# mila-iqia/diffusion_for_multi_scale_molecular_dynamics

Hardware: AMD Instinct MI355X
Metric: sampled structures/sec (1000-step predictor-corrector SDE sampling) (higher is better)
Workload: dtype f32 (per-edge matrix products as split-f16 hi/lo x3 MFMA terms with f32 accumulation: 22-bit products; state, updates, reductions and every other layer in f32)

## Files before the change

### diffusion_for_multi_scale_molecular_dynamics_amd/csrc/mdx_egnn_chain.hip

```cpp
#include <hip/hip_runtime.h>
#include <stdint.h>

#include <type_traits>

#include "../../include/mdx_hip.h"

namespace {

typedef _Float16 half8 __attribute__((ext_vector_type(8)));
typedef _Float16 half2v __attribute__((ext_vector_type(2)));
typedef float f32x16 __attribute__((ext_vector_type(16)));
typedef float f32x4 __attribute__((ext_vector_type(4)));
typedef __attribute__((address_space(3))) char lds_c;
typedef __attribute__((address_space(3))) float lds_f;
typedef __attribute__((address_space(1))) const char gbl_c;

constexpr int kWave = 64;
constexpr int kWaves = 4;
constexpr int kTileEdges = 32 * kWaves;
constexpr int kFastD = 6;
constexpr int kRing = 4;
constexpr int kScaleSlots = MDX_EGNN_CHAIN_MAX_LAYERS + 4;
constexpr int kMaxPositions = MDX_EGNN_CHAIN_MAX_LAYERS + 2;
constexpr int kEnds = kScaleSlots - 1;
// ... 1242 lines not shown
__device__ __forceinline__ float normalize_factor(float r2) { return tanhf(r2) / sqrtf(r2 + 1.0e-16f); }

__global__ __launch_bounds__(256) void egnn_coord_aggregate_kernel(const float* __restrict__ s, const float* __restrict__ coord,
                                                                   const int64_t* __restrict__ edges,
                                                                   const int64_t* __restrict__ offsets,
                                                                   const int64_t* __restrict__ degree, int64_t n_nodes, int D,
                                                                   int mean, int flags, float* __restrict__ out)
{
    const int64_t total = n_nodes * D;
    for (int64_t idx = blockIdx.x * (int64_t)blockDim.x + threadIdx.x; idx < total; idx += (int64_t)gridDim.x * blockDim.x) {
        const int64_t node = idx / D;
        const int k = (int)(idx - node * D);
        const int64_t e0 = offsets[node], deg = degree[node];
        const float ci = coord[idx];
        float acc = 0.0f;
        for (int64_t e = e0; e < e0 + deg; ++e) {
            const int64_t dst = edges[2 * e + 1];
            float diff = ci - coord[dst * D + k];
            if (flags & MDX_EGNN_COORD_NORMALIZE) {
                float r2 = 0.0f;
                for (int j = 0; j < D; ++j) {
                    const float dj = coord[node * D + j] - coord[dst * D + j];
                    r2 += dj * dj;
                }
                diff = normalize_factor(r2) * diff;
            }
            acc += diff * coord_head_value(s[e], flags);
        }
        if (mean && deg > 0) acc = acc / (float)deg;
        out[idx] = ci + acc;
    }
}

__global__ __launch_bounds__(256) void segment_combine_kernel(const float* __restrict__ pieces, const int64_t* __restrict__ offsets,
                                                              const int64_t* __restrict__ degree, int64_t n_nodes, int H,
                                                              int mean, float* __restrict__ out, const float* __restrict__ left,
                                                              int64_t boundary_rows)
{
    const int lane = threadIdx.x % kWave;
    const int64_t wave = (blockIdx.x * (int64_t)blockDim.x + threadIdx.x) / kWave;
    const int64_t n_waves = ((int64_t)gridDim.x * blockDim.x) / kWave;
    const int quads = H >> 2;
    for (int64_t node = wave; node < n_nodes; node += n_waves) {
        const int64_t e0 = offsets[node], deg = degree[node], e1 = e0 + deg;
        const float count = (mean && deg > 0) ? (float)deg : 1.0f;
        const int64_t last_row = ((e1 - 1) & 15) == 15 ? ((e1 - 1) >> 4) : boundary_rows + node;
        for (int q = lane; q < quads; q += kWave) {
            f32x4 acc = {0.0f, 0.0f, 0.0f, 0.0f};
            for (int64_t e = e0 | 15; e < e1 - 1; e += 16) acc += reinterpret_cast<const f32x4*>(pieces + (e >> 4) * H)[q];
            if (deg > 0) acc += reinterpret_cast<const f32x4*>(pieces + last_row * H)[q];
            if (mean) acc = acc / count;
            if (left) {
                reinterpret_cast<f32x4*>(out + node * 2 * H)[q] = reinterpret_cast<const f32x4*>(left + node * H)[q];
                reinterpret_cast<f32x4*>(out + node * 2 * H + H)[q] = acc;
            } else {
                reinterpret_cast<f32x4*>(out + node * H)[q] = acc;
            }
        }
    }
}

__global__ __launch_bounds__(256) void egnn_node_gather_kernel(const float* __restrict__ pieces, const int64_t* __restrict__ offsets,
                                                               const int64_t* __restrict__ degree, int64_t n_nodes, int H,
                                                               int mean_messages, float* __restrict__ out,
                                                               const float* __restrict__ left, int64_t boundary_rows,
                                                               const float* __restrict__ s, const float* __restrict__ coord,
                                                               const int64_t* __restrict__ edges, int D, int mean_coords,
                                                               int flags, float* __restrict__ coord_out)
{
    const int lane = threadIdx.x % kWave;
    const int64_t wave = (blockIdx.x * (int64_t)blockDim.x + threadIdx.x) / kWave;
    const int64_t n_waves = ((int64_t)gridDim.x * blockDim.x) / kWave;
    const int quads = H >> 2;
    for (int64_t node = wave; node < n_nodes; node += n_waves) {
        const int64_t e0 = offsets[node], deg = degree[node], e1 = e0 + deg;
        float part[8] = {0, 0, 0, 0, 0, 0, 0, 0}, ci[8];
#pragma unroll
        for (int k = 0; k < 8; ++k) ci[k] = k < D ? coord[node * D + k] : 0.0f;
        for (int64_t e = e0 + lane; e < e1; e += kWave) {
            const int64_t dst = edges[2 * e + 1];
            const float se = coord_head_value(s[e], flags);
            if (flags & MDX_EGNN_COORD_NORMALIZE) {
                float diff[8], r2 = 0.0f;
#pragma unroll
                for (int k = 0; k < 8; ++k) {
                    diff[k] = k < D ? ci[k] - coord[dst * D + k] : 0.0f;
                    if (k < D) r2 += diff[k] * diff[k];
                }
                const float f = normalize_factor(r2);
#pragma unroll
                for (int k = 0; k < 8; ++k)
                    if (k < D) part[k] += (f * diff[k]) * se;
            } else {
#pragma unroll
                for (int k = 0; k < 8; ++k)
                    if (k < D) part[k] += (ci[k] - coord[dst * D + k]) * se;
            }
        }
        const float count = (mean_messages && deg > 0) ? (float)deg : 1.0f;
        const int64_t last_row = ((e1 - 1) & 15) == 15 ? ((e1 - 1) >> 4) : boundary_rows + node;
        for (int q = lane; pieces && q < quads; q += kWave) {
            f32x4 acc = {0.0f, 0.0f, 0.0f, 0.0f};
            for (int64_t e = e0 | 15; e < e1 - 1; e += 16) acc += reinterpret_cast<const f32x4*>(pieces + (e >> 4) * H)[q];
            if (deg > 0) acc += reinterpret_cast<const f32x4*>(pieces + last_row * H)[q];
            if (mean_messages) acc = acc / count;
            if (left) {
                reinterpret_cast<f32x4*>(out + node * 2 * H)[q] = reinterpret_cast<const f32x4*>(left + node * H)[q];
                reinterpret_cast<f32x4*>(out + node * 2 * H + H)[q] = acc;
            } else {
                reinterpret_cast<f32x4*>(out + node * H)[q] = acc;
            }
        }
#pragma unroll
        for (int k = 0; k < 8; ++k) {
            if (k < D) {
                float v = part[k];
                v += __builtin_bit_cast(float, __builtin_amdgcn_update_dpp(0, __builtin_bit_cast(int, v), 0x111, 0xf, 0xf, false));
                v += __builtin_bit_cast(float, __builtin_amdgcn_update_dpp(0, __builtin_bit_cast(int, v), 0x112, 0xf, 0xf, false));
                v += __builtin_bit_cast(float, __builtin_amdgcn_update_dpp(0, __builtin_bit_cast(int, v), 0x114, 0xf, 0xf, false));
                v += __builtin_bit_cast(float, __builtin_amdgcn_update_dpp(0, __builtin_bit_cast(int, v), 0x118, 0xf, 0xf, false));
                v += __builtin_bit_cast(float, __builtin_amdgcn_update_dpp(0, __builtin_bit_cast(int, v), 0x142, 0xa, 0xf, false));
                v += __builtin_bit_cast(float, __builtin_amdgcn_update_dpp(0, __builtin_bit_cast(int, v), 0x143, 0xc, 0xf, false));
                part[k] = __builtin_bit_cast(float, __builtin_amdgcn_readlane(__builtin_bit_cast(int, v), 63));
            }
        }
        if (lane < D) {
            float total = 0.0f, mine = 0.0f;
#pragma unroll
            for (int k = 0; k < 8; ++k) {
                if (k == lane) { total = part[k]; mine = ci[k]; }
            }
            if (mean_coords && deg > 0) total = total / (float)deg;
            coord_out[node * D + lane] = mine + total;
        }
    }
}

// ... 152 lines not shown
int64_t mdx_egnn_piece_rows(int64_t n_edges, int64_t n_nodes)
{
    if (n_edges < 0 || n_nodes < 0) return -1;
    return ((n_edges + 15) >> 4) + n_nodes;
}

int mdx_segment_combine(const float* pieces, int64_t n_edges, const int64_t* offsets, const int64_t* degree, int64_t n_nodes,
                        int H, int mean, const float* left, float* out, mdx_stream_t stream)
{
    if (n_nodes < 0 || H < 4 || n_edges < 0) return MDX_ERR_INVALID_ARG;
    if (H & 3) return MDX_ERR_UNSUPPORTED;
    if (n_nodes == 0) return MDX_OK;
    if (!pieces || !offsets || !degree || !out) return MDX_ERR_INVALID_ARG;
    int64_t blocks = (n_nodes * kWave + 255) / 256;
    if (blocks > 16384) blocks = 16384;
    hipLaunchKernelGGL(segment_combine_kernel, dim3((unsigned)blocks), dim3(256), 0, reinterpret_cast<hipStream_t>(stream),
                       pieces, offsets, degree, n_nodes, H, mean, out, left, (n_edges + 15) >> 4);
    return hipGetLastError() == hipSuccess ? MDX_OK : MDX_ERR_HIP;
}

int mdx_egnn_node_gather(const float* pieces, int64_t n_edges, const int64_t* offsets, const int64_t* degree, int64_t n_nodes,
                         int H, int mean_messages, const float* left, float* out, const float* edge_scalar, const float* coord,
                         int coord_dimension, const int64_t* edges, int mean_coords, int coord_flags, float* coord_out,
                         mdx_stream_t stream)
{
    if (n_nodes < 0 || H < 4 || n_edges < 0 || coord_dimension < 1) return MDX_ERR_INVALID_ARG;
    if (coord_flags & ~(MDX_EGNN_COORD_NORMALIZE | MDX_EGNN_COORD_TANH)) return MDX_ERR_INVALID_ARG;
    if ((H & 3) || coord_dimension > 8) return MDX_ERR_UNSUPPORTED;
    if (n_nodes == 0) return MDX_OK;
    if (!offsets || !degree || !edge_scalar || !coord || !edges || !coord_out) return MDX_ERR_INVALID_ARG;
    if (pieces ? !out : (out || left)) return MDX_ERR_INVALID_ARG;
    int64_t blocks = (n_nodes * kWave + 255) / 256;
    if (blocks > 16384) blocks = 16384;
    hipLaunchKernelGGL(egnn_node_gather_kernel, dim3((unsigned)blocks), dim3(256), 0, reinterpret_cast<hipStream_t>(stream),
                       pieces, offsets, degree, n_nodes, H, mean_messages, out, left, (n_edges + 15) >> 4, edge_scalar, coord, edges,
                       coord_dimension, mean_coords, coord_flags, coord_out);
    return hipGetLastError() == hipSuccess ? MDX_OK : MDX_ERR_HIP;
}

int mdx_mlp_chain_rows(const mdx_egnn_chain_t* c, const float* x, const float* residual, int64_t n_rows,
                       const int64_t* n_rows_dev, float* out, uint32_t* status, mdx_stream_t stream)
{
    if (!c || n_rows < 0) return MDX_ERR_INVALID_ARG;
    if (c->n_message_layers < 1 || c->n_coord_layers != 0 || (c->precision < 0 || c->precision > 2)) return MDX_ERR_INVALID_ARG;
    if (c->n_message_layers > MDX_EGNN_CHAIN_MAX_LAYERS) return MDX_ERR_UNSUPPORTED;
    if (c->hidden != 32 && c->hidden != 64 && c->hidden != 128 && c->hidden != 256) return MDX_ERR_UNSUPPORTED;
    if (n_rows == 0) return MDX_OK;
    if (!c->weight_image || !c->biases || !x || !out || (c->precision >= 1 && !c->weight_exponents)) return MDX_ERR_INVALID_ARG;
    ChainArgs a{};
    a.image = (const char*)c->weight_image; a.biases = c->biases; a.exps = c->weight_exponents;
    a.act_exps = c->activation_exponents; a.act_max = c->activation_maxima;
    a.n_edges_dev = n_rows_dev; a.n_edges = n_rows; a.n_message = c->n_message_layers; a.n_coord = 0; a.D = 0;
    a.rows_in = x; a.residual = residual; a.rows_out = out; a.status = status; a.ld_in = c->hidden;
    const int layers = a.n_message;
    hipStream_t st = reinterpret_cast<hipStream_t>(stream);
#define MDX_ROWS_CASE(HH)                                                                          \
    case HH: return c->precision == 0 ? launch_chain<HH, 0, 1>(a, layers, st) : (c->precision == 1 ? launch_chain<HH, 1, 1>(a, layers, st) : launch_chain<HH, 2, 1>(a, layers, st));
    switch (c->hidden) {
        MDX_ROWS_CASE(32)
        MDX_ROWS_CASE(64)
        MDX_ROWS_CASE(128)
        MDX_ROWS_CASE(256)
    }
#undef MDX_ROWS_CASE
    return MDX_ERR_UNSUPPORTED;
}

// ... 69 lines not shown
```

### diffusion_for_multi_scale_molecular_dynamics_amd/csrc/mdx_egnn_table.hip

```cpp
#include <hip/hip_runtime.h>
#include <stdint.h>

#include "../../include/mdx_hip.h"
#include "mdx_launch.hpp"

using namespace mdx;

namespace {

typedef float f32x4 __attribute__((ext_vector_type(4)));

__device__ __forceinline__ void lagrange_weights(float t, float w[4])
{
    const float tp = t + 1.0f, tm = t - 1.0f, t2 = t - 2.0f;
    w[0] = -(t * tm * t2) / 6.0f;
    w[1] = (tp * tm * t2) / 2.0f;
    w[2] = -(tp * t * t2) / 2.0f;
    w[3] = (tp * t * tm) / 6.0f;
}

__device__ __forceinline__ float interpolate(const float w[4], float v0, float v1, float v2, float v3)
{
    return ((w[0] * v0 + w[1] * v1) + w[2] * v2) + w[3] * v3;
}

__device__ __forceinline__ f32x4 interpolate4(const float w[4], f32x4 v0, f32x4 v1, f32x4 v2, f32x4 v3)
{
    return ((w[0] * v0 + w[1] * v1) + w[2] * v2) + w[3] * v3;
}

__device__ __forceinline__ float squared_distance(const float* ci, const float* __restrict__ cj, int D)
{
    float r2 = 0.0f;
    for (int k = 0; k < D; ++k) {
        const float dlt = ci[k] - cj[k];
        r2 += dlt * dlt;
    }
    return r2;
}

__device__ __forceinline__ float coord_head_value(float s, int flags) { return (flags & MDX_EGNN_COORD_TANH) ? tanhf(s) : s; }
__device__ __forceinline__ float normalize_factor(float r2) { return tanhf(r2) / sqrtf(r2 + 1.0e-16f); }

__device__ __forceinline__ unsigned abs_bits(float v) { return __float_as_uint(v) & 0x7fffffffu; }

constexpr int kCheckRows = 32;
__global__ __launch_bounds__(256) void egnn_table_check_kernel(const float* __restrict__ messages, const float* __restrict__ scalar,
                                                               int H, int n_pairs, int n_even, unsigned* __restrict__ workspace,
                                                               const uint32_t* __restrict__ table_key,
                                                               const float* __restrict__ sigma)
{
    if (table_is_current(table_key, sigma)) return;
    const int p = blockIdx.x, K = 2 * n_even - 1;
    const int j0 = blockIdx.y * kCheckRows, j1 = min(j0 + kCheckRows, n_even - 2);
    float w[4];
    lagrange_weights(0.5f, w);
    for (int c = threadIdx.x; c <= H; c += blockDim.x) {
        auto value = [&](int row) { return c < H ? messages[((int64_t)p * K + row) * H + c] : scalar[(int64_t)p * K + row]; };
        unsigned err = 0, big = 0;
        for (int j = j0; j < j1; ++j) {
            const float v0 = value(j > 0 ? j - 1 : 1), v1 = value(j), v2 = value(j + 1), v3 = value(j + 2);
            const float mid = value(n_even + j);
            err = max(err, abs_bits(interpolate(w, v0, v1, v2, v3) - mid));
            big = max(big, max(max(abs_bits(v1), abs_bits(v2)), max(abs_bits(v3), abs_bits(mid))));
        }
        if (j0 < j1) {
            atomicMax(workspace + (int64_t)p * (H + 1) + c, err);
            atomicMax(workspace + (int64_t)n_pairs * (H + 1) + p, big);
        }
    }
}
// ... 15 lines not shown
        if (big > 0.0f) mine = fmaxf(mine, err / big);
        else if (err > 0.0f || err != err) mine = INFINITY;
    }
    __syncthreads();
    if (built)
        for (int64_t i = threadIdx.x; i < n_entries + n_pairs; i += blockDim.x) workspace[i] = 0u;
    const int table_fail = fail;
    for (int64_t i = 1 + threadIdx.x; i < n_sigma; i += blockDim.x)
        if (!(sigma[i] == sigma[0])) fail = 1;
    worst[threadIdx.x] = mine;
    bad[threadIdx.x] = fail | (table_fail << 1);
    __syncthreads();
    for (int s = 128; s > 0; s >>= 1) {
        if ((int)threadIdx.x < s) {
            worst[threadIdx.x] = fmaxf(worst[threadIdx.x], worst[threadIdx.x + s]);
            bad[threadIdx.x] |= bad[threadIdx.x + s];
        }
        __syncthreads();
    }
    if (threadIdx.x == 0) {
        if (worst_out && built) worst_out[0] = worst[0];
        if (bad[0] && status) atomicOr(status, MDX_STATUS_EGNN_TABLE);
        if (table_key && built) {
            if (bad[0] & 2) {
                table_key[0] = MDX_EGNN_TABLE_NO_KEY;
            } else {
                table_key[0] = __float_as_uint(sigma[0]);
                table_key[1] = table_key[1] + 1u;
            }
        }
    }
}

__global__ __launch_bounds__(256) void egnn_table_gather_kernel(const float* __restrict__ table, const float* __restrict__ table_scalar,
                                                                int H, int n_classes, int n_even, float inv_spacing,
                                                                const int64_t* __restrict__ atom_types,
                                                                const int64_t* __restrict__ offsets, const int64_t* __restrict__ degree,
                                                                int64_t n_nodes, int mean_messages, float* __restrict__ out,
                                                                const float* __restrict__ left, const float* __restrict__ coord,
                                                                const int64_t* __restrict__ edges, int D, int mean_coords,
                                                                int flags, float* __restrict__ coord_out, uint32_t* __restrict__ status)
{
    const int lane = threadIdx.x % kWave;
    const int64_t wave = (blockIdx.x * (int64_t)blockDim.x + threadIdx.x) / kWave;
    const int64_t n_waves = ((int64_t)gridDim.x * blockDim.x) / kWave;
    const int K = 2 * n_even - 1, quads = H >> 2;
    const bool has_quad = lane < quads;
    bool outside = false;
    for (int64_t node = wave; node < n_nodes; node += n_waves) {
        const int64_t e0 = offsets[node], deg = degree[node], e1 = e0 + deg;
        int64_t a = atom_types[node];
        if (a < 0 || a >= n_classes) { outside = true; a = 0; }
        float part[8] = {0, 0, 0, 0, 0, 0, 0, 0}, ci[8];
#pragma unroll
        for (int k = 0; k < 8; ++k) ci[k] = k < D ? coord[node * D + k] : 0.0f;
        f32x4 acc = {0.0f, 0.0f, 0.0f, 0.0f};
        for (int64_t c0 = e0; c0 < e1; c0 += kWave) {
            const int64_t e = c0 + lane;
            int row = 0, row_left = 0;
            float w[4] = {0, 0, 0, 0};
            if (e < e1) {
                const int64_t dst = edges[2 * e + 1];
                int64_t b = atom_types[dst];
                if (b < 0 || b >= n_classes) { outside = true; b = 0; }
                const float r2 = squared_distance(ci, coord + dst * D, D);
                const float u = sqrtf(r2) * inv_spacing;
                int m = 0;
                float t = 0.0f;
                if (u <= (float)(n_even - 2)) {
                    m = min((int)u, n_even - 3);
                    t = u - (float)m;
                } else {
                    outside = true;
                }
                lagrange_weights(t, w);
                row = (int)(a * n_classes + b) * K + m;
                row_left = m > 0 ? row - 1 : row + 1;
                const float s = coord_head_value(interpolate(w, table_scalar[row_left], table_scalar[row], table_scalar[row + 1],
                                                             table_scalar[row + 2]), flags);
                if (flags & MDX_EGNN_COORD_NORMALIZE) {
                    float diff[8], n2 = 0.0f;
#pragma unroll
                    for (int k = 0; k < 8; ++k) {
                        diff[k] = k < D ? ci[k] - coord[dst * D + k] : 0.0f;
                        if (k < D) n2 += diff[k] * diff[k];
                    }
                    const float f = normalize_factor(n2);
#pragma unroll
                    for (int k = 0; k < 8; ++k)
                        if (k < D) part[k] += (f * diff[k]) * s;
                } else {
#pragma unroll
                    for (int k = 0; k < 8; ++k)
                        if (k < D) part[k] += (ci[k] - coord[dst * D + k]) * s;
                }
            }
            const int n = (int)min<int64_t>(kWave, e1 - c0);
            for (int i = 0; i < n; ++i) {
                const int r = __builtin_amdgcn_readlane(row, i), rl = __builtin_amdgcn_readlane(row_left, i);
                float wi[4];
#pragma unroll
                for (int k = 0; k < 4; ++k)
                    wi[k] = __builtin_bit_cast(float, __builtin_amdgcn_readlane(__builtin_bit_cast(int, w[k]), i));
                if (has_quad) {
                    const f32x4* base = reinterpret_cast<const f32x4*>(table + (int64_t)r * H) + lane;
                    const f32x4 v0 = reinterpret_cast<const f32x4*>(table + (int64_t)rl * H)[lane];
                    acc += interpolate4(wi, v0, base[0], base[quads], base[2 * quads]);
                }
            }
        }
        const float count = (mean_messages && deg > 0) ? (float)deg : 1.0f;
        if (has_quad) {
            if (mean_messages) acc = acc / count;
            if (left) {
                reinterpret_cast<f32x4*>(out + node * 2 * H)[lane] = reinterpret_cast<const f32x4*>(left + node * H)[lane];
                reinterpret_cast<f32x4*>(out + node * 2 * H + H)[lane] = acc;
            } else {
                reinterpret_cast<f32x4*>(out + node * H)[lane] = acc;
            }
        }
#pragma unroll
        for (int k = 0; k < 8; ++k) {
            if (k < D) {
                float v = part[k];
                v += __builtin_bit_cast(float, __builtin_amdgcn_update_dpp(0, __builtin_bit_cast(int, v), 0x111, 0xf, 0xf, false));
                v += __builtin_bit_cast(float, __builtin_amdgcn_update_dpp(0, __builtin_bit_cast(int, v), 0x112, 0xf, 0xf, false));
                v += __builtin_bit_cast(float, __builtin_amdgcn_update_dpp(0, __builtin_bit_cast(int, v), 0x114, 0xf, 0xf, false));
                v += __builtin_bit_cast(float, __builtin_amdgcn_update_dpp(0, __builtin_bit_cast(int, v), 0x118, 0xf, 0xf, false));
                v += __builtin_bit_cast(float, __builtin_amdgcn_update_dpp(0, __builtin_bit_cast(int, v), 0x142, 0xa, 0xf, false));
                v += __builtin_bit_cast(float, __builtin_amdgcn_update_dpp(0, __builtin_bit_cast(int, v), 0x143, 0xc, 0xf, false));
                part[k] = __builtin_bit_cast(float, __builtin_amdgcn_readlane(__builtin_bit_cast(int, v), 63));
            }
        }
        if (lane < D) {
            float total = 0.0f, mine = 0.0f;
#pragma unroll
            for (int k = 0; k < 8; ++k) {
                if (k == lane) { total = part[k]; mine = ci[k]; }
            }
            if (mean_coords && deg > 0) total = total / (float)deg;
// ... 17 lines not shown

int mdx_egnn_table_check_keyed(const float* table, const float* table_scalar, int H, int n_classes, int n_even, const float* sigma,
                               int64_t n_sigma, float tolerance, uint32_t* workspace, float* worst_out, uint32_t* status,
                               uint32_t* table_key, mdx_stream_t stream)
{
    if (H < 1 || n_classes < 1 || n_even < 4 || n_sigma < 1 || !(tolerance >= 0.0f)) return MDX_ERR_INVALID_ARG;
    if (!table || !table_scalar || !sigma || !workspace) return MDX_ERR_INVALID_ARG;
    const int n_pairs = n_classes * n_classes;
    const hipStream_t s = as_stream(stream);
    hipLaunchKernelGGL(egnn_table_check_kernel, dim3((unsigned)n_pairs, (unsigned)((n_even - 2 + kCheckRows - 1) / kCheckRows)),
                       dim3(256), 0, s, table, table_scalar, H, n_pairs, n_even, reinterpret_cast<unsigned*>(workspace),
                       table_key, sigma);
    hipLaunchKernelGGL(egnn_table_verdict_kernel, dim3(1), dim3(256), 0, s, reinterpret_cast<unsigned*>(workspace), n_pairs,
                       H + 1, sigma, n_sigma, tolerance, worst_out, status, table_key);
    return launch_status();
}

int mdx_egnn_table_gather(const float* table, const float* table_scalar, int H, int n_classes, int n_even, float inv_spacing,
                          const int64_t* atom_types, const int64_t* offsets, const int64_t* degree, int64_t n_nodes,
                          int mean_messages, const float* left, float* out, const float* coord, int coord_dimension,
                          const int64_t* edges, int mean_coords, int coord_flags, float* coord_out, uint32_t* status,
                          mdx_stream_t stream)
{
    if (n_nodes < 0 || H < 4 || n_classes < 1 || n_even < 4 || coord_dimension < 1 || !(inv_spacing > 0.0f))
        return MDX_ERR_INVALID_ARG;
    if (coord_flags & ~(MDX_EGNN_COORD_NORMALIZE | MDX_EGNN_COORD_TANH)) return MDX_ERR_INVALID_ARG;
    if ((H & 3) || H > 4 * kWave || coord_dimension > 8) return MDX_ERR_UNSUPPORTED;
    if ((int64_t)n_classes * n_classes * (2 * (int64_t)n_even - 1) * H >= ((int64_t)1 << 31)) return MDX_ERR_UNSUPPORTED;
    if (n_nodes == 0) return MDX_OK;
    if (!table || !table_scalar || !atom_types || !offsets || !degree || !out || !coord || !edges || !coord_out)
        return MDX_ERR_INVALID_ARG;
    int64_t blocks = (n_nodes * kWave + 255) / 256;
    if (blocks > 16384) blocks = 16384;
    hipLaunchKernelGGL(egnn_table_gather_kernel, dim3((unsigned)blocks), dim3(256), 0, as_stream(stream),
                       table, table_scalar, H, n_classes, n_even, inv_spacing, atom_types, offsets, degree, n_nodes, mean_messages,
                       out, left, coord, edges, coord_dimension, mean_coords, coord_flags, coord_out, status);
    return launch_status();
}

}
```

### diffusion_for_multi_scale_molecular_dynamics_amd/models/egnn.py

```python
from typing import Callable, Optional, Tuple

import torch
from torch import nn

from .. import kernels
from ..namespace import AXL


def run_mlp(layers, x: torch.Tensor, fused: bool = False) -> torch.Tensor:
    for layer in layers:
        x = layer(x)
    return x


def segment_sum_sorted(data: torch.Tensor, degree: torch.Tensor) -> torch.Tensor:
    return torch.segment_reduce(data, "sum", lengths=degree, axis=0, unsafe=True)


class LayerDeviceState:
    KINDS = ("edge", "rows", "node")

    def __init__(self):
        self.packs = {kind: {} for kind in self.KINDS}
        self.in_use = {kind: (None, None) for kind in self.KINDS}
# ... 267 lines not shown
                                                table, coords_only)
        assert n_edges is None, "a capacity-sized edge list needs the fused edge chain in every layer"
        count = degree.clamp(min=1).to(h.dtype).unsqueeze(1)

        coord_diff = coord.index_select(0, row) - coord.index_select(0, col)
        radial = (coord_diff ** 2).sum(dim=1, keepdim=True)
        if self.normalize:
            coord_diff = torch.tanh(radial) / torch.sqrt(radial + self.epsilon ** 2) * coord_diff

        messages = self._messages(h, edge_index, radial, fused)

        segments = fused and offsets is not None and messages.shape[1] % 4 == 0
        if segments and self._coord_head_is_plain():
            hidden = run_mlp(list(self.coord_mlp)[:-1], messages, fused)
            coord = coord + kernels.egnn_coord_head(hidden.contiguous(), self.coord_mlp[-1].weight.reshape(-1),
                                                    coord_diff.contiguous(), offsets, degree, self.coords_mean)
        else:
            trans = segment_sum_sorted(coord_diff * run_mlp(self.coord_mlp, messages, fused), degree)
            coord = coord + (trans / count if self.coords_mean else trans)

        if segments:
            agg = kernels.segment_rows(messages.contiguous(), offsets, degree, self.message_mean)
        else:
            agg = segment_sum_sorted(messages, degree)
            if self.message_mean:
                agg = agg / count
        out = run_mlp(self.node_mlp, torch.cat([h, agg], dim=1), fused)
        if self.residual:
            out = h + out
        return out, coord


    def table_applies(self, pack, h, coord) -> bool:
        return (pack is not None and not self.attention and pack.piece_sums_ok and pack.message_width == pack.hidden
                and pack.hidden <= 256 and h.shape[1] == pack.hidden and coord.shape[1] <= 8 and self.status_word is not None
                and h.shape[0] < (1 << 31))

    def _table_gather(self, pack, table, left, coord, edge_index, offsets, degree):
        _, grid_coord, grid_edges = kernels.egnn_table_grid(table.n_classes, table.n_even, coord.shape[1], coord.device)
        memo = table.memo
        values, scalars = kernels.egnn_edge_chain(pack, memo.grid_proj, grid_coord, grid_edges, status=self.status_word,
                                                  memo=memo, sigma=table.sigma)
        self.device_state.table_worst = memo.worst
        kernels.egnn_table_check(values, scalars, table.n_classes, table.n_even, table.sigma, memo.workspace,
                                 worst=memo.worst, status=self.status_word, key=memo.key)
        return kernels.egnn_table_gather(values, scalars, table.n_classes, table.n_even, table.atom_types, offsets, degree,
                                         self.message_mean, left, coord, edge_index, self.coords_mean,
                                         flags=self._coord_flags(), status=self.status_word)

    def _forward_edge_chain(self, pack, h, edge_index, coord, degree, offsets, n_edges=None, node_proj=None, next_layer=None,
                            table=None, coords_only=False):
        coord = coord.contiguous()
        if table is not None and self.table_applies(pack, h, coord):
            def gather(left):
                return self._table_gather(pack, table, left, coord, edge_index, offsets, degree)
            return self._node_part(h, gather, next_layer)
        proj = node_proj if node_proj is not None else torch.nn.functional.linear(h, pack.proj_weight)
        in_kernel = pack.piece_sums_ok and h.shape[0] < (1 << 31)
        messages, edge_scalar = kernels.egnn_edge_chain(pack, proj.contiguous(), coord, edge_index, status=self.status_word,
                                                        n_edges_dev=n_edges, piece_sums=in_kernel)
        padded = pack.message_width != pack.hidden
        if padded:
            coord_out = kernels.egnn_coord_aggregate(edge_scalar, coord, edge_index, offsets, degree, self.coords_mean,
                                                     flags=self._coord_flags())
            agg = (kernels.segment_combine(messages, edge_index.shape[0], offsets, degree, self.message_mean) if in_kernel
                   else kernels.segment_rows(messages, offsets, degree, self.message_mean))
            node_in = torch.cat([h, agg[:, :pack.message_width]], dim=1)
        elif in_kernel and h.shape[1] == messages.shape[1] and coord.shape[1] <= 8:
            if coords_only and not self.attention:
# ... 97 lines not shown
```

### diffusion_for_multi_scale_molecular_dynamics_amd/models/score_networks/egnn_score_network.py

```python
import itertools
import math
from dataclasses import dataclass
from typing import AnyStr, Callable, Dict, Optional, Union

import torch

from ...namespace import AXL, NOISE, NOISY_AXL_COMPOSITION
from ...utils import neighbors
from ..egnn import EGNN
from .score_network import ScoreNetwork, ScoreNetworkParameters


@dataclass(kw_only=True)
class EGNNScoreNetworkParameters(ScoreNetworkParameters):

    architecture: str = "egnn"
    number_of_bloch_wave_shells: int = 1
    message_n_hidden_dimensions: int = 1
    message_hidden_dimensions_size: int = 16
    node_n_hidden_dimensions: int = 1
    node_hidden_dimensions_size: int = 32
    coordinate_n_hidden_dimensions: int = 1
    coordinate_hidden_dimensions_size: int = 32
    residual: bool = True
# ... 42 lines not shown


class EGNNScoreNetwork(ScoreNetwork):

    def __init__(self, hyper_params: EGNNScoreNetworkParameters, edge_builder: Optional[Callable] = None):
        super().__init__(hyper_params)
        hp = hyper_params
        self.number_of_features_per_node = self.num_atom_types + 2
        self.number_of_bloch_wave_shells = hp.number_of_bloch_wave_shells
        k_vectors = positive_bloch_wave_vectors(hp.number_of_bloch_wave_shells, self.spatial_dimension)
        self.register_parameter("bloch_wave_reciprocal_lattice_vectors",
                                torch.nn.Parameter(k_vectors, requires_grad=False))
        self.register_parameter("projection_matrices",
                                torch.nn.Parameter(self._projection_matrices(k_vectors), requires_grad=False))
        assert hp.edges in ("fully_connected", "radial_cutoff"), \
            f"Edges type should be fully_connected or radial_cutoff. Got {hp.edges}"
        self.edges = hp.edges
        self.radial_cutoff = hp.radial_cutoff
        if self.edges == "fully_connected":
            assert self.radial_cutoff is None, "Specifying a radial cutoff is inconsistent with edges=fully_connected."
        else:
            assert type(self.radial_cutoff) is float, \
                "A floating point value for the radial cutoff is needed for edges=radial_cutoff."
        self.drop_duplicate_edges = hp.drop_duplicate_edges
        self.edge_builder = edge_builder
        self.graph_status = None
        self.static_edge_list_max_fraction = 0.5
        self._logged_two_call_switch = False
        self.first_layer_table = "auto"
        self.sigma_uniform_hint = False
        self.first_layer_table_reuse = True
        self.skip_unread_logits = True
        self.logits_unread_hint = False
        self.egnn = self._make_egnn(hp)

    def __getstate__(self):
        state = dict(self.__dict__)
        state.pop("_fully_connected_edges", None)
        state.pop("_table_grid_x", None)
        return state

    @property
    def edge_chain_precision(self):
        return self.egnn.graph_layers[0].edge_chain_precision if len(self.egnn.graph_layers) else None

    @edge_chain_precision.setter
    def edge_chain_precision(self, value):
        for layer in self.egnn.graph_layers:
            layer.edge_chain_precision = value

    def adapt_f16_range(self):
        for layer in self.egnn.graph_layers:
            layer.adapt_f16_range()

    def begin_f16_range_fallback(self):
        for layer in self.egnn.graph_layers:
            layer.begin_f16_range_fallback()

    def reset_f16_range(self):
        for layer in self.egnn.graph_layers:
            layer.reset_f16_range()

    def table_builds(self) -> int:
        return self.egnn.graph_layers[0].table_builds() if len(self.egnn.graph_layers) else 0

    def check_status(self):
        if self.graph_status is not None:
            try:
                neighbors._raise_if_cutoff_too_large(self.graph_status)
            finally:
                self.graph_status.zero_()

    def _impose_non_mask_atomic_type_prediction(self, output: AXL):
        if output.A is not None and not getattr(output.A, "_mdx_mask_imposed", False):
            super()._impose_non_mask_atomic_type_prediction(output)

    def _first_projection_of_inputs(self):
        from ... import kernels
        layers = self.egnn.graph_layers
        if len(layers) == 0 or not layers[0].use_fused_ops:
            return None
        pack = layers[0]._edge_chain_pack()
        emb = self.egnn.embedding_in
        if pack is None or pack.proj_weight.shape[1] != emb.out_features:
            return None
        first = layers[0].message_mlp[0].weight
        stamp = kernels.parameter_stamp(first, emb.weight, emb.bias) + (layers[0].edge_chain_precision,)
        if getattr(self, "_first_projection", (None, None))[0] != stamp:
            with torch.no_grad():
                w2 = (pack.proj_weight.double() @ emb.weight.double()).float().contiguous()
                b2 = (pack.proj_weight.double() @ emb.bias.double()).float().contiguous()
            self._first_projection = (stamp, (w2, b2))
        return self._first_projection[1]

    def _first_layer_table(self, edges, z, h, sigma, atom_types, k_vectors, second):
        from ... import kernels
        mode = self.first_layer_table
        if mode not in ("auto", "on", "off"):
            raise ValueError(f"first_layer_table should be auto, on or off. Got {mode}")
        layer = self.egnn.graph_layers[0]
        if mode != self.__dict__.get("_table_mode_seen", mode):
            layer.reset_table_memos()
        self._table_mode_seen = mode
        if mode == "off" or (mode == "auto" and not self.sigma_uniform_hint):
            return None
        if not layer.table_applies(layer._edge_chain_pack(), h, z):
            return None
        n_classes = self.num_atom_types + 1
        n_even = kernels.egnn_table_points(z.shape[1])
        if mode == "auto" and n_classes ** 2 * (2 * n_even - 1) * 8 > edges.shape[0]:
            return None
        classes, _, _ = kernels.egnn_table_grid(n_classes, n_even, z.shape[1], z.device)
        G = classes.shape[0]
        grid_x = self.__dict__.get("_table_grid_x")
        if grid_x is None or grid_x.shape[1] != G or grid_x.device != z.device:
            grid_x = self._table_grid_x = torch.zeros(1, G, 3, dtype=torch.float32, device=z.device)
        sigma = sigma.to(device=z.device, dtype=torch.float32).reshape(-1).contiguous()
        emb = self.egnn.embedding_in
        stamp = kernels.parameter_stamp(emb.weight, emb.bias, *second)
        memo = layer.table_memo(layer._edge_chain_pack(), n_classes, n_even, emb.out_features, z.shape[1], z.device, stamp)
        if not self.first_layer_table_reuse:
            memo.reset()
        _, _, grid_proj = kernels.egnn_node_inputs(grid_x, k_vectors.contiguous(), sigma, classes.reshape(1, G),
                                                   emb.weight.detach().contiguous(), emb.bias.detach().contiguous(), second=second,
                                                   memo=memo)
        return kernels.EgnnTable(grid_proj=grid_proj, sigma=sigma, atom_types=atom_types.reshape(-1).long().contiguous(),
                                 n_classes=n_classes, n_even=n_even, memo=memo)

    def _make_egnn(self, hp):
        return EGNN(
            input_size=self.number_of_features_per_node, num_classes=self.num_atom_types + 1,
            message_n_hidden_dimensions=hp.message_n_hidden_dimensions,
            message_hidden_dimensions_size=hp.message_hidden_dimensions_size,
            node_n_hidden_dimensions=hp.node_n_hidden_dimensions,
            node_hidden_dimensions_size=hp.node_hidden_dimensions_size,
            coordinate_n_hidden_dimensions=hp.coordinate_n_hidden_dimensions,
            coordinate_hidden_dimensions_size=hp.coordinate_hidden_dimensions_size,
            residual=hp.residual, attention=hp.attention, normalize=hp.normalize, tanh=hp.tanh,
            coords_agg=hp.coords_agg, message_agg=hp.message_agg, n_layers=hp.n_layers)

    @staticmethod
    def _projection_matrices(k_vectors: torch.Tensor) -> torch.Tensor:
        n_k, d = k_vectors.shape
        gamma = torch.zeros(d, 2 * n_k, 2 * n_k)
# ... 46 lines not shown
        if not fits and not self._logged_two_call_switch:
            import logging
            logging.getLogger(__name__).warning(
                "EGNN radius graph: a capacity-sized edge list would take %.1f GB of the %.1f GB free on the device; using "
                "the two-call protocol (one host read per forward, the sampler iteration is not captured in a hipGraph)",
                needed / 2 ** 30, free / 2 ** 30)
            self._logged_two_call_switch = True
        return fits

    def capture_safe(self, batch_size: int, number_of_atoms: int, device) -> bool:
        if self.edges == "fully_connected":
            return True
        if self.edge_builder is not None:
            return False
        return self._static_edge_list_fits(batch_size, number_of_atoms, torch.device(device))

    def _forward_unchecked(self, batch: Dict[AnyStr, torch.Tensor], conditional: bool = False) -> AXL:
        comp = batch[NOISY_AXL_COMPOSITION]
        x = comp.X
        bsz, n, d = x.shape
        if x.is_cuda and (self.graph_status is None or self.graph_status.device != x.device):
            self.graph_status = torch.zeros(1, dtype=torch.int32, device=x.device)
        for layer in self.egnn.graph_layers:
            layer.status_word = self.graph_status if x.is_cuda else None
        edges, degree = self._build_edges(x, comp.L)

        emb = self.egnn.embedding_in
        sigma_in = batch[NOISE]
        if (x.is_cuda and not torch.is_grad_enabled() and d == 3 and x.dtype == torch.float32 and
                emb.in_features == self.num_atom_types + 2 and sigma_in.numel() == bsz):
            from ... import kernels
            k_vectors = self.bloch_wave_reciprocal_lattice_vectors.to(x)
            second = self._first_projection_of_inputs()
            res = kernels.egnn_node_inputs(x.contiguous(), k_vectors.contiguous(),
                                           sigma_in.to(device=x.device, dtype=torch.float32).reshape(-1).contiguous(),
                                           comp.A.reshape(bsz, n).long().contiguous(), emb.weight.detach().contiguous(),
                                           emb.bias.detach().contiguous(), second=second)
            z, h, first_proj = res if second is not None else (res[0], res[1], None)
            table = self._first_layer_table(edges, z, h, sigma_in, comp.A, k_vectors, second) if second is not None else None
            head = self.egnn.node_classification_layer
            if head.out_features <= 8 and head.in_features % 4 == 0 and comp.L.dtype == torch.float32:
                out = self.egnn(h=h, edges=edges, x=z, degree=degree, embedded=True, first_proj=first_proj, classify=False,
                                first_table=table, coords_only=self.skip_unread_logits and self.logits_unread_hint)
                if out.A is None:
                    scores = kernels.egnn_scores(z, out.X.contiguous(), k_vectors.contiguous())
                    return AXL(A=None, X=scores.reshape(bsz, n, d), L=torch.zeros_like(comp.L))
                scores, logits, zeros = kernels.egnn_outputs(
                    z, out.X.contiguous(), k_vectors.contiguous(), out.A.contiguous(), head.weight.detach().contiguous(),
                    head.bias.detach().contiguous(), self.num_atom_types, comp.L.numel())
                logits = logits.reshape(bsz, n, -1)
                logits._mdx_mask_imposed = True
                return AXL(A=logits, X=scores.reshape(bsz, n, d), L=zeros.reshape(comp.L.shape))
            out = self.egnn(h=h, edges=edges, x=z, degree=degree, embedded=True, first_proj=first_proj, first_table=table)
            scores = kernels.egnn_scores(z, out.X.contiguous(), k_vectors.contiguous())
            return AXL(A=out.A.reshape(bsz, n, -1), X=scores.reshape(bsz, n, d), L=torch.zeros_like(comp.L))

        flat = x.reshape(bsz * n, d)
        k_vectors = self.bloch_wave_reciprocal_lattice_vectors.to(flat)
        if flat.is_cuda:
            kr = ((2.0 * math.pi * flat)[:, None, :] * k_vectors[None, :, :]).sum(dim=-1)
        else:
            kr = (2.0 * math.pi * flat) @ k_vectors.t()
        if flat.is_cuda:
            kr64 = kr.double()
            z = torch.stack([kr64.cos().to(kr.dtype), kr64.sin().to(kr.dtype)], dim=2).reshape(bsz * n, -1)
        else:
            z = torch.stack([kr.cos(), kr.sin()], dim=2).reshape(bsz * n, -1)

        sigmas = batch[NOISE].to(x.device).repeat_interleave(n, dim=0)
        one_hot = torch.nn.functional.one_hot(comp.A.reshape(-1).long(), self.num_atom_types + 1).to(x.dtype)
        h = torch.cat([sigmas, one_hot], dim=1)
# ... 9 lines not shown
```

Baseline: 21.64.

## Batch piece loads, specialize gather kernels for D=6, skip dead first projections

```diff
diff --git a/diffusion_for_multi_scale_molecular_dynamics_amd/csrc/mdx_egnn_chain.hip b/diffusion_for_multi_scale_molecular_dynamics_amd/csrc/mdx_egnn_chain.hip
--- a/diffusion_for_multi_scale_molecular_dynamics_amd/csrc/mdx_egnn_chain.hip
+++ b/diffusion_for_multi_scale_molecular_dynamics_amd/csrc/mdx_egnn_chain.hip
@@ -1298,6 +1298,30 @@
     }
 }
 
+constexpr int kPieceDepth = 4;
+
+__device__ __forceinline__ f32x4 sum_pieces(const float* __restrict__ pieces, int H, int q, int64_t e0, int64_t e1, int64_t deg,
+                                            int64_t last_row, int64_t own_row)
+{
+    f32x4 acc = {0.0f, 0.0f, 0.0f, 0.0f};
+    const f32x4 last = reinterpret_cast<const f32x4*>(pieces + (deg > 0 ? last_row : own_row) * H)[q];
+    for (int64_t e = e0 | 15; e < e1 - 1; e += 16 * kPieceDepth) {
+        f32x4 v[kPieceDepth];
+#pragma unroll
+        for (int j = 0; j < kPieceDepth; ++j) {
+            const int64_t ej = e + 16 * j;
+            v[j] = reinterpret_cast<const f32x4*>(pieces + ((ej < e1 - 1 ? ej : e) >> 4) * H)[q];
+        }
+#pragma unroll
+        for (int j = 0; j < kPieceDepth; ++j) {
+            const f32x4 sum = acc + v[j];
+            acc = e + 16 * j < e1 - 1 ? sum : acc;
+        }
+    }
+    const f32x4 sum = acc + last;
+    return deg > 0 ? sum : acc;
+}
+
 __global__ __launch_bounds__(256) void segment_combine_kernel(const float* __restrict__ pieces, const int64_t* __restrict__ offsets,
                                                               const int64_t* __restrict__ degree, int64_t n_nodes, int H,
                                                               int mean, float* __restrict__ out, const float* __restrict__ left,
@@ -1312,9 +1336,7 @@
         const float count = (mean && deg > 0) ? (float)deg : 1.0f;
         const int64_t last_row = ((e1 - 1) & 15) == 15 ? ((e1 - 1) >> 4) : boundary_rows + node;
         for (int q = lane; q < quads; q += kWave) {
-            f32x4 acc = {0.0f, 0.0f, 0.0f, 0.0f};
-            for (int64_t e = e0 | 15; e < e1 - 1; e += 16) acc += reinterpret_cast<const f32x4*>(pieces + (e >> 4) * H)[q];
-            if (deg > 0) acc += reinterpret_cast<const f32x4*>(pieces + last_row * H)[q];
+            f32x4 acc = sum_pieces(pieces, H, q, e0, e1, deg, last_row, boundary_rows + node);
             if (mean) acc = acc / count;
             if (left) {
                 reinterpret_cast<f32x4*>(out + node * 2 * H)[q] = reinterpret_cast<const f32x4*>(left + node * H)[q];
@@ -1326,14 +1348,23 @@
     }
 }
 
+template <int DD>
+__device__ __forceinline__ void load_point(const float* __restrict__ p, int D, float c[8])
+{
+#pragma unroll
+    for (int k = 0; k < 8; ++k) c[k] = k < (DD ? DD : D) ? p[k] : 0.0f;
+}
+
+template <int DD>
 __global__ __launch_bounds__(256) void egnn_node_gather_kernel(const float* __restrict__ pieces, const int64_t* __restrict__ offsets,
                                                                const int64_t* __restrict__ degree, int64_t n_nodes, int H,
                                                                int mean_messages, float* __restrict__ out,
                                                                const float* __restrict__ left, int64_t boundary_rows,
                                                                const float* __restrict__ s, const float* __restrict__ coord,
-                                                               const int64_t* __restrict__ edges, int D, int mean_coords,
+                                                               const int64_t* __restrict__ edges, int D_runtime, int mean_coords,
                                                                int flags, float* __restrict__ coord_out)
 {
+    const int D = DD ? DD : D_runtime;
     const int lane = threadIdx.x % kWave;
     const int64_t wave = (blockIdx.x * (int64_t)blockDim.x + threadIdx.x) / kWave;
     const int64_t n_waves = ((int64_t)gridDim.x * blockDim.x) / kWave;
@@ -1341,18 +1372,19 @@
     for (int64_t node = wave; node < n_nodes; node += n_waves) {
         const int64_t e0 = offsets[node], deg = degree[node], e1 = e0 + deg;
         float part[8] = {0, 0, 0, 0, 0, 0, 0, 0}, ci[8];
-#pragma unroll
-        for (int k = 0; k < 8; ++k) ci[k] = k < D ? coord[node * D + k] : 0.0f;
+        load_point<DD>(coord + node * D, D, ci);
         for (int64_t e = e0 + lane; e < e1; e += kWave) {
             const int64_t dst = edges[2 * e + 1];
             const float se = coord_head_value(s[e], flags);
+            float cj[8], diff[8];
+            load_point<DD>(coord + dst * D, D, cj);
+#pragma unroll
+            for (int k = 0; k < 8; ++k) diff[k] = k < D ? ci[k] - cj[k] : 0.0f;
             if (flags & MDX_EGNN_COORD_NORMALIZE) {
-                float diff[8], r2 = 0.0f;
-#pragma unroll
-                for (int k = 0; k < 8; ++k) {
-                    diff[k] = k < D ? ci[k] - coord[dst * D + k] : 0.0f;
+                float r2 = 0.0f;
+#pragma unroll
+                for (int k = 0; k < 8; ++k)
                     if (k < D) r2 += diff[k] * diff[k];
-                }
                 const float f = normalize_factor(r2);
 #pragma unroll
                 for (int k = 0; k < 8; ++k)
@@ -1360,15 +1392,13 @@
             } else {
 #pragma unroll
                 for (int k = 0; k < 8; ++k)
-                    if (k < D) part[k] += (ci[k] - coord[dst * D + k]) * se;
+                    if (k < D) part[k] += diff[k] * se;
             }
         }
         const float count = (mean_messages && deg > 0) ? (float)deg : 1.0f;
         const int64_t last_row = ((e1 - 1) & 15) == 15 ? ((e1 - 1) >> 4) : boundary_rows + node;
         for (int q = lane; pieces && q < quads; q += kWave) {
-            f32x4 acc = {0.0f, 0.0f, 0.0f, 0.0f};
-            for (int64_t e = e0 | 15; e < e1 - 1; e += 16) acc += reinterpret_cast<const f32x4*>(pieces + (e >> 4) * H)[q];
-            if (deg > 0) acc += reinterpret_cast<const f32x4*>(pieces + last_row * H)[q];
+            f32x4 acc = sum_pieces(pieces, H, q, e0, e1, deg, last_row, boundary_rows + node);
             if (mean_messages) acc = acc / count;
             if (left) {
                 reinterpret_cast<f32x4*>(out + node * 2 * H)[q] = reinterpret_cast<const f32x4*>(left + node * H)[q];
@@ -1587,7 +1617,8 @@
     if (pieces ? !out : (out || left)) return MDX_ERR_INVALID_ARG;
     int64_t blocks = (n_nodes * kWave + 255) / 256;
     if (blocks > 16384) blocks = 16384;
-    hipLaunchKernelGGL(egnn_node_gather_kernel, dim3((unsigned)blocks), dim3(256), 0, reinterpret_cast<hipStream_t>(stream),
+    const auto kernel = coord_dimension == 6 ? egnn_node_gather_kernel<6> : egnn_node_gather_kernel<0>;
+    hipLaunchKernelGGL(kernel, dim3((unsigned)blocks), dim3(256), 0, reinterpret_cast<hipStream_t>(stream),
                        pieces, offsets, degree, n_nodes, H, mean_messages, out, left, (n_edges + 15) >> 4, edge_scalar, coord, edges,
                        coord_dimension, mean_coords, coord_flags, coord_out);
     return hipGetLastError() == hipSuccess ? MDX_OK : MDX_ERR_HIP;
diff --git a/diffusion_for_multi_scale_molecular_dynamics_amd/csrc/mdx_egnn_table.hip b/diffusion_for_multi_scale_molecular_dynamics_amd/csrc/mdx_egnn_table.hip
--- a/diffusion_for_multi_scale_molecular_dynamics_amd/csrc/mdx_egnn_table.hip
+++ b/diffusion_for_multi_scale_molecular_dynamics_amd/csrc/mdx_egnn_table.hip
@@ -27,16 +27,6 @@
 __device__ __forceinline__ f32x4 interpolate4(const float w[4], f32x4 v0, f32x4 v1, f32x4 v2, f32x4 v3)
 {
     return ((w[0] * v0 + w[1] * v1) + w[2] * v2) + w[3] * v3;
-}
-
-__device__ __forceinline__ float squared_distance(const float* ci, const float* __restrict__ cj, int D)
-{
-    float r2 = 0.0f;
-    for (int k = 0; k < D; ++k) {
-        const float dlt = ci[k] - cj[k];
-        r2 += dlt * dlt;
-    }
-    return r2;
 }
 
 __device__ __forceinline__ float coord_head_value(float s, int flags) { return (flags & MDX_EGNN_COORD_TANH) ? tanhf(s) : s; }
@@ -118,28 +108,40 @@
     }
 }
 
-__global__ __launch_bounds__(256) void egnn_table_gather_kernel(const float* __restrict__ table, const float* __restrict__ table_scalar,
+constexpr int kGatherDepth = 1;
+
+template <int DD>
+__device__ __forceinline__ void load_point(const float* __restrict__ p, int D, float c[8])
+{
+#pragma unroll
+    for (int k = 0; k < 8; ++k) c[k] = k < (DD ? DD : D) ? p[k] : 0.0f;
+}
+
+template <int DD>
+__global__ __launch_bounds__(256) __attribute__((amdgpu_waves_per_eu(4)))
+void egnn_table_gather_kernel(const float* __restrict__ table, const float* __restrict__ table_scalar,
                                                                 int H, int n_classes, int n_even, float inv_spacing,
                                                                 const int64_t* __restrict__ atom_types,
                                                                 const int64_t* __restrict__ offsets, const int64_t* __restrict__ degree,
                                                                 int64_t n_nodes, int mean_messages, float* __restrict__ out,
                                                                 const float* __restrict__ left, const float* __restrict__ coord,
-                                                                const int64_t* __restrict__ edges, int D, int mean_coords,
+                                                                const int64_t* __restrict__ edges, int D_runtime, int mean_coords,
                                                                 int flags, float* __restrict__ coord_out, uint32_t* __restrict__ status)
 {
+    const int D = DD ? DD : D_runtime;
     const int lane = threadIdx.x % kWave;
     const int64_t wave = (blockIdx.x * (int64_t)blockDim.x + threadIdx.x) / kWave;
     const int64_t n_waves = ((int64_t)gridDim.x * blockDim.x) / kWave;
     const int K = 2 * n_even - 1, quads = H >> 2;
     const bool has_quad = lane < quads;
+    const f32x4* rows = reinterpret_cast<const f32x4*>(table) + (has_quad ? lane : 0);
     bool outside = false;
     for (int64_t node = wave; node < n_nodes; node += n_waves) {
         const int64_t e0 = offsets[node], deg = degree[node], e1 = e0 + deg;
         int64_t a = atom_types[node];
+        float part[8] = {0, 0, 0, 0, 0, 0, 0, 0}, ci[8];
+        load_point<DD>(coord + node * D, D, ci);
         if (a < 0 || a >= n_classes) { outside = true; a = 0; }
-        float part[8] = {0, 0, 0, 0, 0, 0, 0, 0}, ci[8];
-#pragma unroll
-        for (int k = 0; k < 8; ++k) ci[k] = k < D ? coord[node * D + k] : 0.0f;
         f32x4 acc = {0.0f, 0.0f, 0.0f, 0.0f};
         for (int64_t c0 = e0; c0 < e1; c0 += kWave) {
             const int64_t e = c0 + lane;
@@ -148,8 +150,14 @@
             if (e < e1) {
                 const int64_t dst = edges[2 * e + 1];
                 int64_t b = atom_types[dst];
+                float cj[8], diff[8], r2 = 0.0f;
+                load_point<DD>(coord + dst * D, D, cj);
                 if (b < 0 || b >= n_classes) { outside = true; b = 0; }
-                const float r2 = squared_distance(ci, coord + dst * D, D);
+#pragma unroll
+                for (int k = 0; k < 8; ++k) {
+                    diff[k] = k < D ? ci[k] - cj[k] : 0.0f;
+                    if (k < D) r2 += diff[k] * diff[k];
+                }
                 const float u = sqrtf(r2) * inv_spacing;
                 int m = 0;
                 float t = 0.0f;
@@ -162,36 +170,41 @@
                 lagrange_weights(t, w);
                 row = (int)(a * n_classes + b) * K + m;
                 row_left = m > 0 ? row - 1 : row + 1;
-                const float s = coord_head_value(interpolate(w, table_scalar[row_left], table_scalar[row], table_scalar[row + 1],
-                                                             table_scalar[row + 2]), flags);
+                const float s0 = table_scalar[row_left], s1 = table_scalar[row], s2 = table_scalar[row + 1],
+                            s3 = table_scalar[row + 2];
+                const float s = coord_head_value(interpolate(w, s0, s1, s2, s3), flags);
                 if (flags & MDX_EGNN_COORD_NORMALIZE) {
-                    float diff[8], n2 = 0.0f;
-#pragma unroll
-                    for (int k = 0; k < 8; ++k) {
-                        diff[k] = k < D ? ci[k] - coord[dst * D + k] : 0.0f;
-                        if (k < D) n2 += diff[k] * diff[k];
-                    }
-                    const float f = normalize_factor(n2);
+                    const float f = normalize_factor(r2);
 #pragma unroll
                     for (int k = 0; k < 8; ++k)
                         if (k < D) part[k] += (f * diff[k]) * s;
                 } else {
 #pragma unroll
                     for (int k = 0; k < 8; ++k)
-                        if (k < D) part[k] += (ci[k] - coord[dst * D + k]) * s;
-                }
-            }
-            const int n = (int)min<int64_t>(kWave, e1 - c0);
-            for (int i = 0; i < n; ++i) {
-                const int r = __builtin_amdgcn_readlane(row, i), rl = __builtin_amdgcn_readlane(row_left, i);
-                float wi[4];
-#pragma unroll
-                for (int k = 0; k < 4; ++k)
-                    wi[k] = __builtin_bit_cast(float, __builtin_amdgcn_readlane(__builtin_bit_cast(int, w[k]), i));
-                if (has_quad) {
-                    const f32x4* base = reinterpret_cast<const f32x4*>(table + (int64_t)r * H) + lane;
-                    const f32x4 v0 = reinterpret_cast<const f32x4*>(table + (int64_t)rl * H)[lane];
-                    acc += interpolate4(wi, v0, base[0], base[quads], base[2 * quads]);
+                        if (k < D) part[k] += diff[k] * s;
+                }
+            }
+            const int n = __builtin_amdgcn_readfirstlane((int)min<int64_t>(kWave, e1 - c0));
+            for (int i = 0; i < n; i += kGatherDepth) {
+                f32x4 v[kGatherDepth][4];
+                float wi[kGatherDepth][4];
+#pragma unroll
+                for (int j = 0; j < kGatherDepth; ++j) {
+                    const int from = min(i + j, n - 1);
+                    const int r = __builtin_amdgcn_readlane(row, from), rl = __builtin_amdgcn_readlane(row_left, from);
+#pragma unroll
+                    for (int k = 0; k < 4; ++k)
+                        wi[j][k] = __builtin_bit_cast(float, __builtin_amdgcn_readlane(__builtin_bit_cast(int, w[k]), from));
+                    const f32x4* base = rows + (int64_t)r * quads;
+                    v[j][0] = rows[(int64_t)rl * quads];
+                    v[j][1] = base[0];
+                    v[j][2] = base[quads];
+                    v[j][3] = base[2 * quads];
+                }
+#pragma unroll
+                for (int j = 0; j < kGatherDepth; ++j) {
+                    const f32x4 sum = acc + interpolate4(wi[j], v[j][0], v[j][1], v[j][2], v[j][3]);
+                    acc = i + j < n ? sum : acc;
                 }
             }
         }
@@ -275,9 +288,10 @@
         return MDX_ERR_INVALID_ARG;
     int64_t blocks = (n_nodes * kWave + 255) / 256;
     if (blocks > 16384) blocks = 16384;
-    hipLaunchKernelGGL(egnn_table_gather_kernel, dim3((unsigned)blocks), dim3(256), 0, as_stream(stream),
-                       table, table_scalar, H, n_classes, n_even, inv_spacing, atom_types, offsets, degree, n_nodes, mean_messages,
-                       out, left, coord, edges, coord_dimension, mean_coords, coord_flags, coord_out, status);
+    const auto kernel = coord_dimension == 6 ? egnn_table_gather_kernel<6> : egnn_table_gather_kernel<0>;
+    hipLaunchKernelGGL(kernel, dim3((unsigned)blocks), dim3(256), 0, as_stream(stream), table, table_scalar, H, n_classes, n_even,
+                       inv_spacing, atom_types, offsets, degree, n_nodes, mean_messages, out, left, coord, edges, coord_dimension,
+                       mean_coords, coord_flags, coord_out, status);
     return launch_status();
 }
 
diff --git a/diffusion_for_multi_scale_molecular_dynamics_amd/models/egnn.py b/diffusion_for_multi_scale_molecular_dynamics_amd/models/egnn.py
--- a/diffusion_for_multi_scale_molecular_dynamics_amd/models/egnn.py
+++ b/diffusion_for_multi_scale_molecular_dynamics_amd/models/egnn.py
@@ -323,9 +323,12 @@
 
 
     def table_applies(self, pack, h, coord) -> bool:
+        return self.table_applies_to(pack, h.shape[0], h.shape[1], coord.shape[1])
+
+    def table_applies_to(self, pack, n_nodes: int, width: int, coord_dimension: int) -> bool:
         return (pack is not None and not self.attention and pack.piece_sums_ok and pack.message_width == pack.hidden
-                and pack.hidden <= 256 and h.shape[1] == pack.hidden and coord.shape[1] <= 8 and self.status_word is not None
-                and h.shape[0] < (1 << 31))
+                and pack.hidden <= 256 and width == pack.hidden and coord_dimension <= 8 and self.status_word is not None
+                and n_nodes < (1 << 31))
 
     def _table_gather(self, pack, table, left, coord, edge_index, offsets, degree):
         _, grid_coord, grid_edges = kernels.egnn_table_grid(table.n_classes, table.n_even, coord.shape[1], coord.device)
diff --git a/diffusion_for_multi_scale_molecular_dynamics_amd/models/score_networks/egnn_score_network.py b/diffusion_for_multi_scale_molecular_dynamics_amd/models/score_networks/egnn_score_network.py
--- a/diffusion_for_multi_scale_molecular_dynamics_amd/models/score_networks/egnn_score_network.py
+++ b/diffusion_for_multi_scale_molecular_dynamics_amd/models/score_networks/egnn_score_network.py
@@ -98,6 +98,7 @@
         self.first_layer_table_reuse = True
         self.skip_unread_logits = True
         self.logits_unread_hint = False
+        self.skip_dead_projections = True
         self.egnn = self._make_egnn(hp)
 
     def __getstate__(self):
@@ -159,23 +160,32 @@
             self._first_projection = (stamp, (w2, b2))
         return self._first_projection[1]
 
-    def _first_layer_table(self, edges, z, h, sigma, atom_types, k_vectors, second):
+    def _table_selected(self, n_edge_rows: int, n_nodes: int, width: int, coord_dimension: int) -> bool:
         from ... import kernels
         mode = self.first_layer_table
         if mode not in ("auto", "on", "off"):
             raise ValueError(f"first_layer_table should be auto, on or off. Got {mode}")
+        if mode == "off" or (mode == "auto" and not self.sigma_uniform_hint):
+            return False
+        layer = self.egnn.graph_layers[0]
+        if not layer.table_applies_to(layer._edge_chain_pack(), n_nodes, width, coord_dimension):
+            return False
+        n_classes = self.num_atom_types + 1
+        n_even = kernels.egnn_table_points(coord_dimension)
+        return not (mode == "auto" and n_classes ** 2 * (2 * n_even - 1) * 8 > n_edge_rows)
+
+    def _first_layer_table(self, edges, z, h, sigma, atom_types, k_vectors, second):
+        from ... import kernels
+        mode = self.first_layer_table
+        selected = self._table_selected(edges.shape[0], h.shape[0], h.shape[1], z.shape[1])
         layer = self.egnn.graph_layers[0]
         if mode != self.__dict__.get("_table_mode_seen", mode):
             layer.reset_table_memos()
         self._table_mode_seen = mode
-        if mode == "off" or (mode == "auto" and not self.sigma_uniform_hint):
-            return None
-        if not layer.table_applies(layer._edge_chain_pack(), h, z):
+        if not selected:
             return None
         n_classes = self.num_atom_types + 1
         n_even = kernels.egnn_table_points(z.shape[1])
-        if mode == "auto" and n_classes ** 2 * (2 * n_even - 1) * 8 > edges.shape[0]:
-            return None
         classes, _, _ = kernels.egnn_table_grid(n_classes, n_even, z.shape[1], z.device)
         G = classes.shape[0]
         grid_x = self.__dict__.get("_table_grid_x")
@@ -288,11 +298,13 @@
             from ... import kernels
             k_vectors = self.bloch_wave_reciprocal_lattice_vectors.to(x)
             second = self._first_projection_of_inputs()
+            dead = (second is not None and self.skip_dead_projections and
+                    self._table_selected(edges.shape[0], bsz * n, emb.out_features, 2 * k_vectors.shape[0]))
             res = kernels.egnn_node_inputs(x.contiguous(), k_vectors.contiguous(),
                                            sigma_in.to(device=x.device, dtype=torch.float32).reshape(-1).contiguous(),
                                            comp.A.reshape(bsz, n).long().contiguous(), emb.weight.detach().contiguous(),
-                                           emb.bias.detach().contiguous(), second=second)
-            z, h, first_proj = res if second is not None else (res[0], res[1], None)
+                                           emb.bias.detach().contiguous(), second=None if dead else second)
+            z, h, first_proj = res if len(res) == 3 else (res[0], res[1], None)
             table = self._first_layer_table(edges, z, h, sigma_in, comp.A, k_vectors, second) if second is not None else None
             head = self.egnn.node_classification_layer
             if head.out_features <= 8 and head.in_features % 4 == 0 and comp.L.dtype == torch.float32:
```

Result: no change. 21.79, median of 6 (+0.7%).
